# jseppanen/azalea

Measured on AMD Instinct MI355X. Metric: mcts_sims_per_sec, higher is better.
Workload: dtype f16x3 (fp32 operands split hi+lo f16, fp32 accumulate)

## Files before the change

### azalea_amd/csrc/net_kernels.hip

```cpp
#include "net_priv.h"

#ifndef AZX_NET_ABLATE
#define AZX_NET_ABLATE 0
#endif
#ifndef AZX_SAT_TRACK
#define AZX_SAT_TRACK 1
#endif

#include <cmath>
#include <cstdio>
#include <cstdlib>
#include <cstring>
#include <map>
#include <string>
#include <type_traits>
#include <vector>

typedef float f32x16 __attribute__((ext_vector_type(16)));

static thread_local std::string g_net_err;
const char *azx_net_error() { return g_net_err.c_str(); }

int azx_net_fail(int code, const char *msg) {
    g_net_err = msg;
// ... 82 lines not shown
            }
            const float4 *wt = wl + (size_t)tap * (C / 8) * NT * 64;
#pragma unroll 2
            for (int q = 0; q < C / 8; ++q) {
                float4 bfrag[NTW];
#pragma unroll
                for (int n = 0; n < NTW; ++n)
                    bfrag[n] = wt[((size_t)q * NT + (ns * NTW + n)) * 64 + lane];
                float4 afrag[MTW];
#pragma unroll
                for (int m = 0; m < MTW; ++m)
                    afrag[m] = *reinterpret_cast<const float4 *>(src + aoff[m] + 8 * q);
#pragma unroll
                for (int m = 0; m < MTW; ++m)
#pragma unroll
                    for (int n = 0; n < NTW; ++n) {
                        acc[m][n] = __builtin_amdgcn_mfma_f32_32x32x2f32(afrag[m].x, bfrag[n].x, acc[m][n], 0, 0, 0);
                        acc[m][n] = __builtin_amdgcn_mfma_f32_32x32x2f32(afrag[m].y, bfrag[n].y, acc[m][n], 0, 0, 0);
                        acc[m][n] = __builtin_amdgcn_mfma_f32_32x32x2f32(afrag[m].z, bfrag[n].z, acc[m][n], 0, 0, 0);
                        acc[m][n] = __builtin_amdgcn_mfma_f32_32x32x2f32(afrag[m].w, bfrag[n].w, acc[m][n], 0, 0, 0);
                    }
            }
        }
        const bool residual = (layer & 1) != 0;
#pragma unroll
        for (int n = 0; n < NTW; ++n) {
            const int co = (ns * NTW + n) * 32 + li;
            const float bb = P.bias[layer * C + co];
#pragma unroll
            for (int m = 0; m < MTW; ++m) {
#pragma unroll
                for (int r = 0; r < 16; ++r) {
                    const int row = (ms * MTW + m) * 32 + (r & 3) + 8 * (r >> 2) + 4 * lh;
                    if (row < ncells) {
                        float v = acc[m][n][r] + bb;
                        if (residual) v += dst[row * LDW + co];
                        dst[row * LDW + co] = fmaxf(v, 0.0f);
                    }
                }
            }
        }
        __syncthreads();
    }

    for (int b = 0; b < BPB; ++b) {
        const int e = e0 + b;
        if (e >= n_eval) break;
        const float *Xb = lds + (size_t)b * 2 * rows * LDW;
        float4 *out = reinterpret_cast<float4 *>(act_out + (size_t)e * ncells * C);
        for (int idx = tid; idx < ncells * (C / 4); idx += 256) {
            const int pos = idx / (C / 4), c4 = idx - pos * (C / 4);
            out[idx] = *reinterpret_cast<const float4 *>(Xb + pos * LDW + 4 * c4);
        }
    }
}


typedef _Float16 f16x8 __attribute__((ext_vector_type(8)));

__device__ __forceinline__ void split_f16(float v, _Float16 &hi, _Float16 &lo) {
    hi = (_Float16)v;
    lo = (_Float16)(v - (float)hi);
}
__device__ __forceinline__ void split2_f16(float a, float b, uint32_t &hpk, uint32_t &lpk) {
    float la, lb;
    asm("v_cvt_pk_f16_f32 %0, %1, %2" : "=v"(hpk) : "v"(a), "v"(b));
    asm("v_fma_mix_f32 %0, %1, -1.0, %2 op_sel_hi:[1,0,0]" : "=v"(la) : "v"(hpk), "v"(a));
    asm("v_fma_mix_f32 %0, %1, -1.0, %2 op_sel:[1,0,0] op_sel_hi:[1,0,0]" : "=v"(lb) : "v"(hpk), "v"(b));
    asm("v_cvt_pk_f16_f32 %0, %1, %2" : "=v"(lpk) : "v"(la), "v"(lb));
#if AZX_LO_BITS < 10
    lpk = (lpk + LO_RND * 0x10001u) & (LO_MASK * 0x10001u);
#endif
}

#ifdef AZX_NET_STAMP
__device__ unsigned long long g_tower_stamp[10];
#define NT_DECL unsigned long long nt_last = __builtin_amdgcn_s_memtime(), nt_acc[8] = {0, 0, 0, 0, 0, 0, 0, 0}; const unsigned long long nt_rt0 = __builtin_amdgcn_s_memrealtime();
__device__ unsigned long long g_tower_trace[3 * 32768];
#define NT_MARK(r) { const unsigned long long nt_now = __builtin_amdgcn_s_memtime(); nt_acc[r] += nt_now - nt_last; nt_last = nt_now; }
#define NT_FLUSH if (tid == 0) { for (int r_ = 0; r_ < 7; ++r_) atomicAdd(&g_tower_stamp[r_], nt_acc[r_]); atomicAdd(&g_tower_stamp[7], 1ull); atomicAdd(&g_tower_stamp[8], __builtin_amdgcn_s_memrealtime() - nt_rt0); \
    if (blockIdx.x < 32768) { const unsigned hw = __builtin_amdgcn_s_getreg((31 << 11) | 4), xc = __builtin_amdgcn_s_getreg((31 << 11) | 20); \
        g_tower_trace[3 * blockIdx.x] = ((unsigned long long)(xc & 0xf) << 8) | (((hw >> 13) & 7) << 5) | (((hw >> 12) & 1) << 4) | ((hw >> 8) & 0xf); \
        g_tower_trace[3 * blockIdx.x + 1] = nt_rt0; g_tower_trace[3 * blockIdx.x + 2] = __builtin_amdgcn_s_memrealtime(); } }
__device__ unsigned long long g_wide_stamp[10];
#define WT_FLUSH if (lane == 0) { for (int r_ = 0; r_ < 7; ++r_) atomicAdd(&g_wide_stamp[r_], nt_acc[r_]); atomicAdd(&g_wide_stamp[7], 1ull); \
    atomicAdd(&g_wide_stamp[8], __builtin_amdgcn_s_memrealtime() - nt_rt0); }
#else
#define NT_DECL
#define NT_MARK(r)
#define NT_FLUSH
#define WT_FLUSH
#endif

#ifndef F16X3_BPB
#define F16X3_BPB 2
#endif
#ifndef AZX_S16_FENCE
#define AZX_S16_FENCE 1
#endif
typedef float f32x4 __attribute__((ext_vector_type(4)));

__global__ __launch_bounds__(F16X3_BPB * 128, 2) void k_tower_f16x3_s16(NetDev P, const uint8_t *__restrict__ ev_board,
                                                                        const int32_t *__restrict__ n_eval_ptr,
                                                                        int n_eval_host, float *__restrict__ act_out,
                                                                        float *__restrict__ hfeat) {
    constexpr int C = 64, ROWB = 272, MT = 4, NT = 4;
    extern __shared__ __align__(16) unsigned char smem[];
    const int n_eval = n_eval_ptr ? *n_eval_ptr : n_eval_host;
    const int e0 = blockIdx.x * F16X3_BPB;
    if (e0 >= n_eval) return;
    const int tid = threadIdx.x, lane = tid & 63, wave = __builtin_amdgcn_readfirstlane(tid >> 6);
    NT_DECL
    const int wb = wave >> 1, wh = wave & 1;
    const int N = P.N, ncells = P.ncells;
    const int e = e0 + wb;
    const bool live = e < n_eval;
    const int board_b = 128 * ROWB;
    const int zero_off = 0;
    const int x_off = 2 * ROWB + wb * board_b;
    unsigned char *X = smem + x_off;
    const int li = lane & 15, lh = lane >> 4;
    const int lrow = li < 8 ? li ^ 4 : li;
    const int lchunk = 128 * (lh & 1) + 16 * (lh >> 1);

    unsigned long long tapok = 0ull;
    int rbase[MT], ry_[MT], rx_[MT];
#pragma unroll
    for (int m = 0; m < MT; ++m) {
        const int r = 64 * wh + 16 * m + lrow;
        const int ry = r / N, rx = r - ry * N;
        ry_[m] = ry;
        rx_[m] = rx;
        rbase[m] = x_off + r * ROWB + lchunk;
#pragma unroll
        for (int tap = 0; tap < 9; ++tap) {
            const int yy = ry + tap / 3 - 1, xx = rx + tap % 3 - 1;
            if (r < ncells && yy >= 0 && yy < N && xx >= 0 && xx < N) tapok |= 1ull << (tap * 4 + m);
        }
    }
    uint32_t tapok_lo = (uint32_t)tapok, tapok_hi = (uint32_t)(tapok >> 32);
    auto act_offset = [&](int tap, int m) -> int {
        const int delta = ((tap / 3 - 1) * N + (tap % 3 - 1)) * ROWB;
        const uint32_t word = tap < 8 ? tapok_lo : tapok_hi;
        const int mask = (int)(word << (31 - ((tap * 4 + m) & 31))) >> 31;
        return (mask | 0xF0) & (rbase[m] + delta);
    };

    f32x4 res[MT][NT];
    auto load_bias = [&](const float *bias, float4 (&b4)[NT]) {
#pragma unroll
        for (int n = 0; n < NT; ++n) b4[n] = *reinterpret_cast<const float4 *>(bias + 16 * n + 4 * lh);
    };
    float satmax = 0.f;
    auto epilogue = [&](f32x4 (&acc)[MT][NT], const float4 (&bias4)[NT], auto kind_tag) {
        constexpr int kind = decltype(kind_tag)::value;
#pragma unroll
        for (int n = 0; n < NT; ++n) {
            const float4 b4 = bias4[n];
            const float bv[4] = {b4.x, b4.y, b4.z, b4.w};
#pragma unroll
            for (int m = 0; m < MT; ++m) {
                float v4[4];
#pragma unroll
                for (int j = 0; j < 4; ++j) {
                    float v = acc[m][n][j] + bv[j];
                    if (kind == 1) v += res[m][n][j];
                    v = fmaxf(v, 0.0f);
                    if (kind != 0) res[m][n][j] = v;
                    v4[j] = v;
                }
                if (AZX_SAT_TRACK) satmax = fmaxf(fmaxf(satmax, v4[0]), fmaxf(v4[1], fmaxf(v4[2], v4[3])));
                uint2 h4, l4;
                split2_f16(v4[0], v4[1], h4.x, l4.x);
                split2_f16(v4[2], v4[3], h4.y, l4.y);
                unsigned char *pw = X + (64 * wh + 16 * m + lrow) * ROWB + 128 * (lh >> 1) + 16 * n + 8 * (lh & 1);
                *reinterpret_cast<uint2 *>(pw) = h4;
                *reinterpret_cast<uint2 *>(pw + 64) = l4;
            }
        }
    };

    {
        const int NH = N + 2;
        unsigned char *cells = X + 121 * ROWB;
        const uint8_t *bd = ev_board + (size_t)(live ? e : n_eval - 1) * AZX_CELL_STRIDE;
        if (wh == 0) {
            for (int i = lane; i < NH * NH; i += 64) {
                const int y = i / NH - 1, x = i - (y + 1) * NH - 1;
                cells[i] = (y >= 0 && y < N && x >= 0 && x < N) ? bd[y * N + x] : (uint8_t)3;
            }
        }
        for (int i = tid; i < 2 * ROWB / 4; i += F16X3_BPB * 128) reinterpret_cast<uint32_t *>(smem + zero_off)[i] = 0u;
        __syncthreads();
        f32x4 acc[MT][NT];
#pragma unroll
        for (int m = 0; m < MT; ++m)
#pragma unroll
            for (int n = 0; n < NT; ++n) acc[m][n] = f32x4{0.f, 0.f, 0.f, 0.f};
        const uint4 *ws = reinterpret_cast<const uint4 *>(P.Ws16);
        f16x8 wfh[NT], wfl[NT];
#pragma unroll
        for (int n = 0; n < NT; ++n) {
            const uint4 qh = ws[(n * 2) * 64 + lane], ql = ws[(n * 2 + 1) * 64 + lane];
            wfh[n] = *reinterpret_cast<const f16x8 *>(&qh);
            wfl[n] = *reinterpret_cast<const f16x8 *>(&ql);
        }
#pragma unroll
        for (int m = 0; m < MT; ++m) {
            uint32_t onehot = 0u;
            if (64 * wh + 16 * m + lrow < ncells) {
                const unsigned char *c0 = cells + ry_[m] * NH + rx_[m];
#pragma unroll
                for (int tap = 0; tap < 9; ++tap) {
                    const uint32_t v = c0[(tap / 3) * NH + tap % 3];
                    onehot |= (v < 3u ? 1u : 0u) << (3 * tap + v);
                }
            }
            const uint32_t byte = (onehot >> (8 * lh)) & 0xffu;
            uint4 q;
            q.x = ((byte >> 0) & 1u) * 0x3C00u | ((byte >> 1) & 1u) * 0x3C000000u;
            q.y = ((byte >> 2) & 1u) * 0x3C00u | ((byte >> 3) & 1u) * 0x3C000000u;
            q.z = ((byte >> 4) & 1u) * 0x3C00u | ((byte >> 5) & 1u) * 0x3C000000u;
            q.w = ((byte >> 6) & 1u) * 0x3C00u | ((byte >> 7) & 1u) * 0x3C000000u;
            const f16x8 xf = *reinterpret_cast<const f16x8 *>(&q);
#pragma unroll
            for (int n = 0; n < NT; ++n) {
                acc[m][n] = __builtin_amdgcn_mfma_f32_16x16x32_f16(wfh[n], xf, acc[m][n], 0, 0, 0);
                acc[m][n] = __builtin_amdgcn_mfma_f32_16x16x32_f16(wfl[n], xf, acc[m][n], 0, 0, 0);
            }
        }
        float4 sb4[NT];
        load_bias(P.stem_b, sb4);
        __syncthreads();
        epilogue(acc, sb4, std::integral_constant<int, 2>{});
    }
    __syncthreads();
    NT_MARK(0)

    const uint4 *wsrc = reinterpret_cast<const uint4 *>(P.Wh16);
    int stage = 0;
    const int last_stage = P.layers * 18 - 1;
    f16x8 wh_[NT], wl_[NT];
    auto load_w = [&](int st, int nn, int part) {
        const uint4 qq = wsrc[(size_t)min(st, last_stage) * 512 + (nn * 2 + part) * 64 + lane];
        if (part) wl_[nn] = *reinterpret_cast<const f16x8 *>(&qq);
        else wh_[nn] = *reinterpret_cast<const f16x8 *>(&qq);
    };
#pragma unroll
    for (int i = 0; i < 4; ++i) load_w(0, i >> 1, i & 1);
    auto conv_layer = [&](int layer, auto residual_tag) {
        constexpr bool residual = decltype(residual_tag)::value;
        asm volatile("" : "+v"(tapok_lo), "+v"(tapok_hi), "+v"(rbase[0]), "+v"(rbase[1]), "+v"(rbase[2]), "+v"(rbase[3]));
        f32x4 acc[MT][NT];
#pragma unroll
        for (int m = 0; m < MT; ++m)
#pragma unroll
            for (int n = 0; n < NT; ++n) acc[m][n] = f32x4{0.f, 0.f, 0.f, 0.f};
        f16x8 xh[MT], xl[MT];
        auto load_x = [&](int tt, int mm, int part) {
            const unsigned char *pa = smem + act_offset(tt >> 1, mm) + (tt & 1) * 32 + part * 64;
            if (part) xl[mm] = *reinterpret_cast<const f16x8 *>(pa);
            else xh[mm] = *reinterpret_cast<const f16x8 *>(pa);
        };
#pragma unroll
        for (int m = 0; m < MT - 1; ++m) { load_x(0, m, 0); load_x(0, m, 1); }
#pragma unroll
        for (int t = 0; t < 18; ++t) {
#pragma unroll
            for (int h = 0; h < 2; ++h) {
#pragma unroll
                for (int q = 0; q < 24; ++q) {
                    const int m = q / 6, n = 2 * h + (q % 6) / 3, p = q % 3;
                    if (q == 1 || q == 4 || q == 7 || q == 10) {
                        const int idx = (q - 1) / 3;
                        if (h == 0) load_w(stage + t, 2 + (idx >> 1), idx & 1);
                        else load_w(stage + t + 1, idx >> 1, idx & 1);
                    } else if (h == 0 && (q == 13 || q == 16)) {
                        load_x(t, MT - 1, q == 16);
                    } else if (h == 1 && q >= 8 && (q % 6 == 2 || q % 6 == 5)) {
                        if (t + 1 < 18) load_x(t + 1, q / 6 - 1, q % 6 == 5);
                    }
                    const f16x8 wv = p == 1 ? wl_[n] : wh_[n];
                    const f16x8 xv = p == 2 ? xl[m] : xh[m];
                    acc[m][n] = __builtin_amdgcn_mfma_f32_16x16x32_f16(wv, xv, acc[m][n], 0, 0, 0);
#if AZX_S16_FENCE == 2
                    __builtin_amdgcn_sched_barrier(0);
#elif AZX_S16_FENCE == 1
                    if (q % 3 == 2) __builtin_amdgcn_sched_barrier(0);
#elif AZX_S16_FENCE == 3
                    if (q % 6 == 5) __builtin_amdgcn_sched_barrier(0);
#elif AZX_S16_FENCE == 4
                    if (q % 2 == 1) __builtin_amdgcn_sched_barrier(0);
#endif
                }
            }
        }
        stage += 18;
        float4 lb4[NT];
        load_bias(P.bias + layer * C, lb4);
        NT_MARK(2)
        __syncthreads();
        NT_MARK(3)
        epilogue(acc, lb4, std::integral_constant<int, residual ? 1 : 0>{});
        NT_MARK(4)
        __syncthreads();
        NT_MARK(5)
    };
    for (int blk = 0; blk < P.blocks; ++blk) {
        conv_layer(2 * blk, std::false_type{});
        conv_layer(2 * blk + 1, std::true_type{});
    }

    if (hfeat != nullptr) {
        const uint4 *whd = reinterpret_cast<const uint4 *>(P.Whd16);
        f16x8 ah[2], al[2];
#pragma unroll
        for (int ks = 0; ks < 2; ++ks) {
            const uint4 qh = whd[(ks * 2) * 64 + lane], ql = whd[(ks * 2 + 1) * 64 + lane];
            ah[ks] = *reinterpret_cast<const f16x8 *>(&qh);
            al[ks] = *reinterpret_cast<const f16x8 *>(&ql);
        }
        const float4 hb = *reinterpret_cast<const float4 *>(P.hbias16 + 4 * lh);
        const float hbv[4] = {hb.x, hb.y, hb.z, hb.w};
#pragma unroll
        for (int m = 0; m < MT; ++m) {
            f32x4 hacc = f32x4{0.f, 0.f, 0.f, 0.f};
#pragma unroll
            for (int ks = 0; ks < 2; ++ks) {
                const unsigned char *pa = smem + rbase[m] + ks * 32;
                const f16x8 xh = *reinterpret_cast<const f16x8 *>(pa), xl = *reinterpret_cast<const f16x8 *>(pa + 64);
                hacc = __builtin_amdgcn_mfma_f32_16x16x32_f16(ah[ks], xh, hacc, 0, 0, 0);
                hacc = __builtin_amdgcn_mfma_f32_16x16x32_f16(al[ks], xh, hacc, 0, 0, 0);
                hacc = __builtin_amdgcn_mfma_f32_16x16x32_f16(ah[ks], xl, hacc, 0, 0, 0);
            }
            const int row = 64 * wh + 16 * m + lrow;
            if (live && row < ncells) {
#pragma unroll
                for (int r = 0; r < 4; ++r) {
                    const int o = 4 * lh + r;
                    if (o < 6) hfeat[((size_t)e * 6 + o) * ncells + row] = fmaxf(hacc[r] + hbv[r], 0.0f);
                }
            }
        }
    }
    if (live && act_out != nullptr) {
        float *out = act_out + (size_t)e * ncells * C;
#pragma unroll
        for (int m = 0; m < MT; ++m) {
            const int row = 64 * wh + 16 * m + lrow;
            if (row < ncells) {
#pragma unroll
                for (int n = 0; n < NT; ++n)
                    *reinterpret_cast<float4 *>(out + row * C + 16 * n + 4 * lh) =
                        make_float4(res[m][n][0], res[m][n][1], res[m][n][2], res[m][n][3]);
            }
        }
    }
    if (satmax > 65504.0f) atomicOr(P.sat_flag, 1u);
    NT_MARK(6)
    NT_FLUSH
}

#define WIDE_ROWB 272
#define WIDE_MW 3
#define WIDE_NW 2

#ifndef WIDE_STAGE_GROUP
#define WIDE_STAGE_GROUP 6
#endif
#ifndef AZX_WIDE_ABLATE
#define AZX_WIDE_ABLATE 0
#endif

#define WIDE16_MT 6
#define WIDE16_NT 4
struct WideBwdFuse { const unsigned char *mask; const float *raw, *skip; const double *sums; float invN; unsigned int *gmax; };
template <int TRAIN, int NTW = WIDE16_NT>
__device__ __forceinline__ void conv_wide_s16_body(const NetDev &P, int layer, const unsigned short *__restrict__ in,
                                                   unsigned short *out, const unsigned short *resid,
                                                   float *__restrict__ out32,
                                                   const int32_t *__restrict__ n_eval_ptr, int n_eval_host,
                                                   int e_base, int e_end, float unscale, float2 *__restrict__ stat,
                                                   const WideBwdFuse &F = WideBwdFuse{}) {
    constexpr int MT = WIDE16_MT, NT = NTW, ROWB = WIDE_ROWB;
    static_assert(NT == 4 || (NT == 2 && TRAIN != 0), "two tiles per wave: training instantiations only");
    float satmax = 0.f;
    extern __shared__ __align__(16) unsigned char smem[];
    const int n_eval = n_eval_ptr ? *n_eval_ptr : n_eval_host;
    const int C = P.C, N = P.N, ncells = P.ncells;
    const int NCH = C / 64, NT16 = C / 16;
    NT_DECL
    const int e = e_base + blockIdx.y * 8 + (blockIdx.x & 7);
    if (e >= n_eval || e >= e_end) return;
    const int co_base = (blockIdx.x >> 3) * (32 * NT);
    const int tid = threadIdx.x, lane = tid & 63, wave = tid >> 6;
    const int wm = wave & 1, wn = wave >> 1;
    const int row0 = wm ? 80 : 0;
    const int li = lane & 15, lh = lane >> 4;
    const size_t rowg = (size_t)C * 4;
    const unsigned char *gin = reinterpret_cast<const unsigned char *>(in) + (size_t)e * ncells * rowg;
    constexpr int IMG0 = 2 * ROWB;
    const int lrow = li < 8 ? li ^ 4 : li;
    const int lchunk = 128 * (lh & 1) + 16 * (lh >> 1);

    unsigned long long tapok = 0ull;
    int rbase[MT];
#pragma unroll
    for (int m = 0; m < MT; ++m) {
        const int r = row0 + 16 * m + lrow;
        const int ry = r / N, rx = r - ry * N;
        rbase[m] = IMG0 + r * ROWB + lchunk;
#pragma unroll
        for (int tap = 0; tap < 9; ++tap) {
            const int yy = ry + tap / 3 - 1, xx = rx + tap % 3 - 1;
            if (r < ncells && yy >= 0 && yy < N && xx >= 0 && xx < N) tapok |= 1ull << (tap * 6 + m);
        }
    }
    uint32_t tapok_lo = (uint32_t)tapok & 0x3fffffffu, tapok_hi = (uint32_t)(tapok >> 30);
    auto act_offset = [&](int tap, int m) -> int {
        const int delta = ((tap / 3 - 1) * N + (tap % 3 - 1)) * ROWB;
        const uint32_t word = tap < 5 ? tapok_lo : tapok_hi;
        const int bit = (tap < 5 ? tap : tap - 5) * 6 + m;
        const int mask = (int)(word << (31 - bit)) >> 31;
        return (mask | 0xF0) & (rbase[m] + delta);
    };
    if (tid < IMG0 / 4) reinterpret_cast<uint32_t *>(smem)[tid] = 0u;

    auto chan0 = [&](int np) -> int { return co_base + 16 * NT * wn + 32 * np + 8 * lh; };
    f32x4 acc[MT][NT];
    if constexpr (TRAIN != 0) {
#pragma unroll
        for (int m = 0; m < MT; ++m)
#pragma unroll
            for (int n = 0; n < NT; ++n) acc[m][n] = f32x4{0.f, 0.f, 0.f, 0.f};
    } else {
        const unsigned char *gres0 = resid ? reinterpret_cast<const unsigned char *>(resid) + (size_t)e * ncells * rowg : nullptr;
#if AZX_WIDE_ABLATE & 16
        gres0 = nullptr;
#endif
        float bv[2][8];
#pragma unroll
        for (int np = 0; np < 2; ++np) {
            const float4 b0 = *reinterpret_cast<const float4 *>(P.bias + (size_t)layer * C + chan0(np));
// ... 864 lines not shown
            if (b < nb) logit_out[(size_t)(e0 + b) * AZX_CELL_STRIDE + t] = logit;
        }
    }
    __syncthreads();
    if (tid < nb) {
        float acc = 0.f;
        for (int i = 0; i < 64; ++i) acc += h2[i][tid] * P.fc3w[i];
        value_out[e0 + tid] = tanhf(acc + P.fc3b[0]);
    }
    if (!prior_out) return;
    const int lane = tid & 63, wave = tid >> 6;
    for (int b = wave; b < nb; b += 3 * HEADS_KSPLIT) {
        const int e = e0 + b;
        float x[3];
        bool legal[3];
        float mx = -INFINITY;
#pragma unroll
        for (int s = 0; s < 3; ++s) {
            const int cell = s * 64 + lane;
            legal[s] = cell < ncells && ev_board[(size_t)e * AZX_CELL_STRIDE + cell] == 0;
            x[s] = legal[s] ? lg[b][cell] : -INFINITY;
            mx = fmaxf(mx, x[s]);
        }
        mx = wave_max(mx);
        float sum = 0.f;
#pragma unroll
        for (int s = 0; s < 3; ++s) sum += legal[s] ? expf(x[s] - mx) : 0.f;
        const float lse = mx + logf(wave_sum(sum));
        const int flip = ev_flip[e];
#pragma unroll
        for (int s = 0; s < 3; ++s) {
            const int cell = s * 64 + lane;
            if (cell < ncells) {
                const int uc = (flip & 2) ? ncells - 1 - cell : cell;
                int oc = uc;
                if (flip & 1) {
                    const int i = uc / N, j = uc - i * N;
                    oc = (N - 1 - j) * N + (N - 1 - i);
                }
                prior_out[(size_t)e * AZX_CELL_STRIDE + oc] = legal[s] ? expf(x[s] - lse) : 0.f;
            }
        }
    }
}



static int raise_lds_limits() {
    const int cap = 160 * 1024;
    const void *fns[] = {(const void *)k_tower_f16x3_s16, (const void *)k_conv_wide_f16x3_s16,
                         (const void *)k_tower_mfma<64, 4, 2, 1, 2>, (const void *)k_tower_mfma<64, 6, 1, 2, 2>,
                         (const void *)k_tower_mfma<32, 6, 2, 2, 1>, (const void *)k_heads_mfma, (const void *)k_heads};
    for (const void *f : fns)
        if (hipFuncSetAttribute(f, hipFuncAttributeMaxDynamicSharedMemorySize, cap) != hipSuccess)
            return nfail(AZX_EHIP, "net: raising a tower kernel's dynamic LDS limit failed");
    return AZX_OK;
}

int azx_net_create(AzxNet **out, int N, int blocks, int chans, int max_evals, hipStream_t st) {
    if (N < 2 || N > AZX_MAX_BOARD) return nfail(AZX_EINVAL, "net: board size out of range");
    if (blocks < 0 || chans < 1) return nfail(AZX_EINVAL, "net: bad num_blocks/base_chans");
    if (int rc = raise_lds_limits()) return rc;
    AzxNet *net = new AzxNet();
    memset(&net->d, 0, sizeof net->d);
    net->d.N = N;
    net->d.ncells = N * N;
    net->d.C = chans;
    net->d.blocks = blocks;
    net->d.layers = 2 * blocks;
    net->max_evals = max_evals;
    net->stream = st;
    const int ncells = N * N;
    const char *force = getenv("AZX_TOWER");
    const bool want_fp32 = force && !strcmp(force, "fp32");
    if (chans == 64 && ncells <= 121 && blocks >= 1 && !want_fp32) net->tower_variant = 4;
    else if (chans == 64 && ncells <= 128) net->tower_variant = 1;
    else if (chans == 64 && ncells <= 192) net->tower_variant = 2;
    else if (chans == 32 && ncells <= 192) net->tower_variant = 3;
    else if (chans % 128 == 0 && ncells <= 192 && !want_fp32) net->tower_variant = 5;
    net->use_mfma = net->tower_variant != 0;
    { const char *v = getenv("AZX_WIDE_STREAMS"); net->opt_wsplit = std::min(4, std::max(1, v ? atoi(v) : 2)); }
    { const char *v = getenv("AZX_HEADS"); net->opt_heads_mfma = !(v && !strcmp(v, "valu")); }
    { const char *v = getenv("AZX_PACK"); net->pack_on_host = v && !strcmp(v, "host"); }
    {
        char b[260];
        const char *tower = "k_stem_generic + k_conv_generic (VALU)";
        if (net->tower_variant == 4) tower = "k_tower_f16x3_s16";
        else if (net->tower_variant == 5) tower = "k_stem_wide_f16x3 + k_conv_wide_f16x3_s16 per layer";
        else if (net->tower_variant == 1) tower = "k_tower_mfma<64,4,2,1,2> (fp32 MFMA)";
        else if (net->tower_variant == 2) tower = "k_tower_mfma<64,6,1,2,2> (fp32 MFMA)";
        else if (net->tower_variant == 3) tower = "k_tower_mfma<32,6,2,2,1> (fp32 MFMA)";
        const bool hm = net->tower_variant == 4 && net->opt_heads_mfma && ncells <= 128;
        snprintf(b, sizeof b, "%s + %s (%dx%d on %dx%d; AZX_TOWER=%s AZX_WIDE_STREAMS=%d AZX_HEADS=%s AZX_PACK=%s)",
                 tower, hm ? "k_heads_mfma" : "k_heads", blocks, chans, N, N, want_fp32 ? "fp32" : "default",
                 net->opt_wsplit, net->opt_heads_mfma ? "mfma" : "valu", net->pack_on_host ? "host" : "device");
        net->info = b;
    }
    const size_t E = max_evals;
    net->act = nalloc<float>(net, E * ncells * chans);
    net->logit = nalloc<float>(net, E * AZX_CELL_STRIDE);
    if (net->tower_variant == 4) net->hfeat = nalloc<float>(net, E * 6 * ncells);
    net->hb_board = nalloc<uint8_t>(net, E * AZX_CELL_STRIDE);
    net->hb_flip = nalloc<int32_t>(net, E);
    net->hb_value = nalloc<float>(net, E);
    if (!net->use_mfma) {
        net->act2 = nalloc<float>(net, E * ncells * chans);
        net->act3 = nalloc<float>(net, E * ncells * chans);
    }
    if (net->tower_variant == 5) {
        net->wideX = nalloc<unsigned short>(net, E * ncells * chans * 2);
        net->wideY = nalloc<unsigned short>(net, E * ncells * chans * 2);
    }
    if (!net->act || !net->logit || !net->hb_board || !net->hb_flip || !net->hb_value ||
        (!net->use_mfma && (!net->act2 || !net->act3)) || (net->tower_variant == 5 && (!net->wideX || !net->wideY))) {
        azx_net_destroy(net);
        return nfail(AZX_ENOMEM, "net: hipMalloc failed");
    }
    const int bpb = net->tower_variant == 2 ? 1 : 2;
    net->lds_bytes = (size_t)bpb * 2 * (ncells + 1) * (chans + 4) * sizeof(float);
    if (net->tower_variant == 4) net->lds_bytes = (size_t)F16X3_BPB * 128 * 272 + 2 * 272;
    if (net->tower_variant == 5) net->lds_bytes = (size_t)(ncells + 2) * WIDE_ROWB;
    net->d.sat_flag = nalloc<uint32_t>(net, 4);
    if (!net->d.sat_flag || hipDeviceSynchronize() != hipSuccess) {
        azx_net_destroy(net);
        return nfail(AZX_ENOMEM, "net: hipMalloc failed");
    }
    *out = net;
    return AZX_OK;
}

void azx_net_set_stream(AzxNet *net, hipStream_t st, const uint32_t *mask, int words) {
    if (!net) return;
    for (int i = 0; i < 3; ++i) {
        if (net->stream2[i]) { (void)hipStreamSynchronize(net->stream2[i]); (void)hipStreamDestroy(net->stream2[i]); }
        if (net->ev_join[i]) (void)hipEventDestroy(net->ev_join[i]);
        net->stream2[i] = nullptr;
        net->ev_join[i] = nullptr;
    }
    if (net->ev_fork) (void)hipEventDestroy(net->ev_fork);
    net->ev_fork = nullptr;
    net->streams_ok = false;
    net->cu_mask.assign(mask, mask + (mask ? words : 0));
    net->stream = st;
}

void azx_net_destroy(AzxNet *net) {
    if (net) {
        for (int i = 0; i < 3; ++i) {
            if (net->stream2[i]) { (void)hipStreamSynchronize(net->stream2[i]); (void)hipStreamDestroy(net->stream2[i]); }
            if (net->ev_join[i]) (void)hipEventDestroy(net->ev_join[i]);
            net->stream2[i] = nullptr;
            net->ev_join[i] = nullptr;
        }
        if (net->ev_fork) (void)hipEventDestroy(net->ev_fork);
        net->ev_fork = nullptr;
    }
#ifdef AZX_NET_STAMP
    {
        unsigned long long h[10] = {0};
        if (hipMemcpyFromSymbol(h, HIP_SYMBOL(g_wide_stamp), sizeof h) == hipSuccess && h[7]) {
            static const char *nm[6] = {"prologue (bias + residual, setup)", "barrier after staging", "k-loops (MFMA)", "epilogue (stores acknowledged)",
                                        "barrier before staging (skew)", "staging: requests, round trips, LDS writes"};
            unsigned long long tot = 0;
            for (int r = 0; r < 6; ++r) tot += h[r];
            fprintf(stderr, "k_conv_wide_f16x3_s16 stamps over %llu waves: %.0f cycles/wave, shader clock %.0f MHz during the kernel\n",
                    h[7], (double)tot / h[7], h[8] ? 100.0 * (double)tot / (double)h[8] : 0.0);
            for (int r = 0; r < 6; ++r)
                fprintf(stderr, "  %-44s %6.1f%%  %9.0f cycles/wave\n", nm[r], 100.0 * h[r] / tot, (double)h[r] / h[7]);
            unsigned long long z[10] = {0};
            (void)hipMemcpyToSymbol(HIP_SYMBOL(g_wide_stamp), z, sizeof z);
        }
    }
    {
        unsigned long long h[10] = {0};
        if (hipMemcpyFromSymbol(h, HIP_SYMBOL(g_tower_stamp), sizeof h) == hipSuccess && h[7]) {
            static const char *nm[7] = {"stem", "residual load/setup", "k-loop (MFMA)", "barrier after k-loop",
                                        "epilogue", "barrier after epilogue", "output store"};
            unsigned long long tot = 0;
            for (int r = 0; r < 7; ++r) tot += h[r];
            fprintf(stderr, "k_tower_f16x3_s16 stamps over %llu blocks: %.0f cycles/block, shader clock %.0f MHz during the kernel\n",
                    h[7], (double)tot / h[7], h[8] ? 100.0 * (double)tot / (double)h[8] : 0.0);
            for (int r = 0; r < 7; ++r)
                fprintf(stderr, "  %-24s %6.1f%%  %9.0f cycles/block\n", nm[r], 100.0 * h[r] / tot, (double)h[r] / h[7]);
            {
                std::vector<unsigned long long> tr(3 * 32768);
                (void)hipMemcpyFromSymbol(tr.data(), HIP_SYMBOL(g_tower_trace), tr.size() * sizeof(unsigned long long));
                std::map<unsigned long long, std::vector<std::pair<unsigned long long, unsigned long long>>> cu;
                unsigned long long t0 = ~0ull, t1 = 0;
                size_t nblk = 0;
                for (int b = 0; b < 32768; ++b)
                    if (tr[3 * b + 2]) {
                        cu[tr[3 * b]].push_back({tr[3 * b + 1], tr[3 * b + 2]});
                        t0 = std::min(t0, tr[3 * b + 1]);
                        t1 = std::max(t1, tr[3 * b + 2]);
                        ++nblk;
                    }
                double busy = 0, mn = 1e30, mx = 0, lastend_min = 1e30, lastend_max = 0;
                size_t cmin = 1 << 30, cmax = 0;
                for (auto &kv : cu) {
                    double b = 0, le = 0;
                    for (auto &iv : kv.second) { b += (double)(iv.second - iv.first); le = std::max(le, (double)(iv.second - t0)); }
                    busy += b; mn = std::min(mn, b); mx = std::max(mx, b);
                    cmin = std::min(cmin, kv.second.size()); cmax = std::max(cmax, kv.second.size());
                    lastend_min = std::min(lastend_min, le); lastend_max = std::max(lastend_max, le);
                }
                fprintf(stderr, "  last launch: %zu blocks on %zu CUs, span %.1f us, blocks/CU %zu..%zu, mean resident blocks/CU %.2f, "
                        "per-CU block-time %.0f..%.0f us, CU finish %.0f..%.0f us\n", nblk, cu.size(), (t1 - t0) / 100.0, cmin, cmax,
                        busy / ((double)(t1 - t0) * cu.size()), mn / 100.0, mx / 100.0, lastend_min / 100.0, lastend_max / 100.0);
            }
            int nb = -1;
            (void)hipOccupancyMaxActiveBlocksPerMultiprocessor(&nb, (const void *)k_tower_f16x3_s16, F16X3_BPB * 128, net->lds_bytes);
            hipFuncAttributes fa;
            memset(&fa, 0, sizeof fa);
            (void)hipFuncGetAttributes(&fa, (const void *)k_tower_f16x3_s16);
            fprintf(stderr, "  runtime occupancy: %d blocks/CU (dynamic LDS %zu B, static %zu B, %d VGPRs, max threads %d)\n", nb,
                    net->lds_bytes, (size_t)fa.sharedSizeBytes, fa.numRegs, fa.maxThreadsPerBlock);
        }
    }
#endif
    if (!net) return;
    for (void *p : net->allocs) (void)hipFree(p);
    if (net->raw_tab_host) (void)hipHostFree((void *)net->raw_tab_host);
    if (net->wmax_host) (void)hipHostFree((void *)net->wmax_host);
    delete net;
}

bool azx_net_ready(const AzxNet *net) { return net && net->ready; }


static void run_net(AzxNet *net, const uint8_t *boards, const int32_t *flip, const int32_t *n_eval_ptr,
                    int n_host, int max_n, float *logit, float *value, float *prior, hipStream_t st, size_t row0 = 0) {
    const NetDev &d = net->d;
    if (max_n <= 0) return;
    const size_t act_rows = row0 * d.ncells * d.C;
    float *const act = net->act + act_rows;
    float *const act2 = net->act2 ? net->act2 + act_rows : nullptr;
    float *const act3 = net->act3 ? net->act3 + act_rows : nullptr;
    float *const hfeat_rows = net->hfeat ? net->hfeat + row0 * 6 * d.ncells : nullptr;
    const float *hfeat = nullptr;
    if (net->use_mfma) {
        const size_t lds = net->lds_bytes;
        if (net->tower_variant == 4) {
            const dim3 grid((max_n + F16X3_BPB - 1) / F16X3_BPB), block(F16X3_BPB * 128);
            hipLaunchKernelGGL(k_tower_f16x3_s16, grid, block, lds, st, d, boards, n_eval_ptr, n_host, (float *)nullptr, hfeat_rows);
            hfeat = hfeat_rows;
        } else if (net->tower_variant == 5) {
            const dim3 grid(max_n, d.C / 128), block(256);
            hipLaunchKernelGGL(k_stem_wide_f16x3, grid, block, 0, st, d, boards, net->wideX,
                               d.blocks == 0 ? net->act : (float *)nullptr, n_eval_ptr, n_host);
            const int wsplit = net->opt_wsplit;
            {
                int parts = wsplit;
                if (parts > 1 && !net->ev_fork) {
                    bool ok = hipEventCreateWithFlags(&net->ev_fork, hipEventDisableTiming) == hipSuccess;
                    for (int i = 0; i < 3 && ok; ++i)
                        ok = (net->cu_mask.empty() ? hipStreamCreateWithFlags(&net->stream2[i], hipStreamNonBlocking)
                                                   : hipExtStreamCreateWithCUMask(&net->stream2[i], (uint32_t)net->cu_mask.size(), net->cu_mask.data())) == hipSuccess &&
                             hipEventCreateWithFlags(&net->ev_join[i], hipEventDisableTiming) == hipSuccess;
                    net->streams_ok = ok;
                }
                if (parts > 1 && !net->streams_ok) parts = 1;
                const int per = (((max_n + parts - 1) / parts + 7) / 8) * 8;
                if (per >= max_n) parts = 1;
                if (parts > 1 && hipEventRecord(net->ev_fork, st) != hipSuccess) parts = 1;
                for (int part = 1; part < parts; ++part)
                    if (hipStreamWaitEvent(net->stream2[part - 1], net->ev_fork, 0) != hipSuccess) { parts = 1; break; }
                const int per_ok = parts > 1 ? per : max_n;
                for (int part = 0; part < parts; ++part) {
                    hipStream_t s = part ? net->stream2[part - 1] : st;
                    const int e0 = part * per_ok, e1 = std::min(max_n, e0 + per_ok);
                    if (e1 <= e0) continue;
                    const dim3 g(8 * (d.C / 128), (e1 - e0 + 7) / 8);
                    for (int b = 0; b < d.blocks; ++b) {
                        hipLaunchKernelGGL(k_conv_wide_f16x3_s16, g, block, lds, s, d, 2 * b, (const unsigned short *)net->wideX, net->wideY,
                                           (const unsigned short *)nullptr, (float *)nullptr, n_eval_ptr, n_host, e0, e1);
                        hipLaunchKernelGGL(k_conv_wide_f16x3_s16, g, block, lds, s, d, 2 * b + 1, (const unsigned short *)net->wideY, net->wideX,
                                           (const unsigned short *)net->wideX, b == d.blocks - 1 ? net->act : (float *)nullptr, n_eval_ptr, n_host, e0, e1);
                    }
                    if (part) {
                        if (hipEventRecord(net->ev_join[part - 1], s) != hipSuccess ||
                            hipStreamWaitEvent(st, net->ev_join[part - 1], 0) != hipSuccess)
                            (void)hipStreamSynchronize(s);
                    }
                }
            }
        } else if (net->tower_variant == 1) {
            hipLaunchKernelGGL((k_tower_mfma<64, 4, 2, 1, 2>), dim3((max_n + 1) / 2), dim3(256), lds, st, d, boards, n_eval_ptr, n_host, act);
        } else if (net->tower_variant == 2) {
            hipLaunchKernelGGL((k_tower_mfma<64, 6, 1, 2, 2>), dim3(max_n), dim3(256), lds, st, d, boards, n_eval_ptr, n_host, act);
        } else {
            hipLaunchKernelGGL((k_tower_mfma<32, 6, 2, 2, 1>), dim3((max_n + 1) / 2), dim3(256), lds, st, d, boards, n_eval_ptr, n_host, act);
        }
    } else {
        const int grid = 2048;
        hipLaunchKernelGGL(k_stem_generic, dim3(grid), dim3(256), 0, st, d, boards, n_eval_ptr, n_host, max_n, act);
        float *x = act, *y = act2, *z = act3;
        for (int b = 0; b < d.blocks; ++b) {
            hipLaunchKernelGGL(k_conv_generic, dim3(grid), dim3(256), 0, st, d, 2 * b, x, (const float *)nullptr, n_eval_ptr, n_host, max_n, y);
            hipLaunchKernelGGL(k_conv_generic, dim3(grid), dim3(256), 0, st, d, 2 * b + 1, y, x, n_eval_ptr, n_host, max_n, z);
            std::swap(x, z);
        }
        if (x != act)
            (void)hipMemcpyAsync(act, x, (size_t)max_n * d.ncells * d.C * sizeof(float), hipMemcpyDeviceToDevice, st);
    }
    if (hfeat != nullptr && net->opt_heads_mfma && d.ncells <= 128) {
        const size_t hl = std::max((size_t)HM_MB * d.hm_lda, (size_t)HM_MB * AZX_CELL_STRIDE + (size_t)HM_MB * 64) * sizeof(float);
        hipLaunchKernelGGL(k_heads_mfma, dim3((max_n + HM_MB - 1) / HM_MB), dim3(256), hl, st, d, hfeat, boards, flip, n_eval_ptr, n_host, logit, value, prior);
    } else {
        const size_t hl = ((size_t)(6 * d.ncells + 64) * HEADS_BPB + (size_t)HEADS_BPB * AZX_CELL_STRIDE +
                           (size_t)(HEADS_KSPLIT - 1) * (64 + 192) * HEADS_BPB) * sizeof(float);
        hipLaunchKernelGGL(k_heads, dim3((max_n + HEADS_BPB - 1) / HEADS_BPB), dim3(192 * HEADS_KSPLIT), hl, st, d, act, hfeat, boards, flip, n_eval_ptr, n_host, logit, value, prior);
    }
}

const char *azx_net_kernel_info(const AzxNet *net) { return net->info.c_str(); }

int azx_net_check_range(AzxNet *net, hipStream_t st) {
    if (!net || !net->d.sat_flag) return AZX_OK;
    uint32_t flag = 0;
    if (hipMemcpyAsync(&flag, net->d.sat_flag, sizeof flag, hipMemcpyDeviceToHost, st) != hipSuccess ||
        hipStreamSynchronize(st) != hipSuccess)
        return nfail(AZX_EHIP, "net: reading the activation range flag failed");
    if (!flag) return AZX_OK;
    (void)hipMemsetAsync(net->d.sat_flag, 0, sizeof flag, st);
    return nfail(AZX_ERANGE, "net: an activation of the residual tower exceeded the f16 range (65504) of the split-f16 "
                             "kernels -- the evaluations of this call are not valid (AZX_TOWER=fp32 runs the fp32 MFMA tower)");
}
// ... 79 lines not shown
```

### azalea_amd/csrc/net_priv.h

```cpp
#pragma once
#include <hip/hip_runtime.h>
#include <stdint.h>

#include <algorithm>
#include <string>
#include <vector>

#include "net.h"

struct NetDev {
    int N, ncells, C, blocks, layers;
    const float *stemT;
    const float *stem_b;
    const unsigned short *Ws;
    const unsigned short *Ws16, *Wh16;
    const unsigned short *Whd16;
    const float *hbias16;
    const float *Wp;
    const float *Wg;
    const float *bias;
    const float *wv, *bv;
    const float *wp, *bp;
    const float *fc2T, *fc2b;
    const float *fc3w, *fc3b;
    const float *mfcT, *mfcb;
    const float *hmP, *hmV;
    int hm_lda;
    uint32_t *sat_flag;
};

#ifndef AZX_LO_BITS
#define AZX_LO_BITS 10
#endif
#define LO_MASK ((0xFFFFu << (10 - AZX_LO_BITS)) & 0xFFFFu)
#define LO_RND (AZX_LO_BITS < 10 ? (1u << (9 - AZX_LO_BITS)) : 0u)
static inline unsigned short lo_round_bits(unsigned short bits) {
    return (unsigned short)((bits + LO_RND) & LO_MASK);
}

struct AzxNet {
    NetDev d;
    int max_evals = 0;
    bool ready = false;
    bool use_mfma = false;
    hipStream_t stream = nullptr;
    std::vector<void *> allocs;
    float *act = nullptr, *act2 = nullptr, *act3 = nullptr;
    unsigned short *wideX = nullptr, *wideY = nullptr;
    float *logit = nullptr;
    float *hfeat = nullptr;
    uint8_t *hb_board = nullptr;
    int32_t *hb_flip = nullptr;
    float *hb_value = nullptr;
    size_t lds_bytes = 0;
    int tower_variant = 0;
    hipStream_t stream2[3] = {nullptr, nullptr, nullptr};
    std::vector<uint32_t> cu_mask;
    hipEvent_t ev_fork = nullptr, ev_join[3] = {nullptr, nullptr, nullptr};
    bool streams_ok = false;
    int opt_wsplit = 2;
    bool opt_heads_mfma = true;
    std::string info;
    bool pack_on_host = false;
    bool packed_once = false;
    const float **raw_tab = nullptr;
    const float **raw_tab_host = nullptr;
    int raw_slots = 0;
    float *raw_arena = nullptr;
    size_t raw_arena_floats = 0;
    double *fold = nullptr;
    uint32_t *wmax = nullptr;
    uint32_t *wmax_host = nullptr;
    struct PackBuf { std::string name; void *ptr; size_t bytes; };
    std::vector<PackBuf> packs;
};

int azx_net_fail(int code, const char *msg);

template <typename T>
static T *nalloc(AzxNet *net, size_t count) {
    void *p = nullptr;
    if (hipMalloc(&p, std::max<size_t>(count * sizeof(T), 16)) != hipSuccess) return nullptr;
    (void)hipMemset(p, 0, std::max<size_t>(count * sizeof(T), 16));
    net->allocs.push_back(p);
    return reinterpret_cast<T *>(p);
}
```

Baseline: 5.158 million.

## Skip dead-tap MFMAs for last row tile and rebalance wave roles by LDS slot

In the fused f16x3 tower kernel, the last row tile's MFMA triples for the bottom three taps (t>=12) are wrapped in inline asm with a wave-uniform branch. The branch skips them when a ballot shows none of those taps are valid for the wave's rows, so waves covering off-board rows stop doing zero work. It also adds a role flip of the wave-half assignment, chosen by reading the LDS base hardware register, to balance skipped work across SIMDs. The inline asm bypasses compiler scheduling and adds manual nops at the drain point, and a debug placement trace is added under the stamp build.

```diff
diff --git a/azalea_amd/csrc/net_kernels.hip b/azalea_amd/csrc/net_kernels.hip
--- a/azalea_amd/csrc/net_kernels.hip
+++ b/azalea_amd/csrc/net_kernels.hip
@@ -188,6 +188,9 @@
     if (blockIdx.x < 32768) { const unsigned hw = __builtin_amdgcn_s_getreg((31 << 11) | 4), xc = __builtin_amdgcn_s_getreg((31 << 11) | 20); \
         g_tower_trace[3 * blockIdx.x] = ((unsigned long long)(xc & 0xf) << 8) | (((hw >> 13) & 7) << 5) | (((hw >> 12) & 1) << 4) | ((hw >> 8) & 0xf); \
         g_tower_trace[3 * blockIdx.x + 1] = nt_rt0; g_tower_trace[3 * blockIdx.x + 2] = __builtin_amdgcn_s_memrealtime(); } }
+__device__ unsigned int g_tower_place[4 * 32768];
+#define NT_PLACE if (lane == 0 && blockIdx.x < 32768) g_tower_place[4 * blockIdx.x + wave] = 0x80000000u | \
+    (__builtin_amdgcn_s_getreg((11 << 11) | 6) << 8) | ((__builtin_amdgcn_s_getreg((31 << 11) | 4) >> 4) & 3u);
 __device__ unsigned long long g_wide_stamp[10];
 #define WT_FLUSH if (lane == 0) { for (int r_ = 0; r_ < 7; ++r_) atomicAdd(&g_wide_stamp[r_], nt_acc[r_]); atomicAdd(&g_wide_stamp[7], 1ull); \
     atomicAdd(&g_wide_stamp[8], __builtin_amdgcn_s_memrealtime() - nt_rt0); }
@@ -195,6 +198,7 @@
 #define NT_DECL
 #define NT_MARK(r)
 #define NT_FLUSH
+#define NT_PLACE
 #define WT_FLUSH
 #endif
 
@@ -205,11 +209,18 @@
 #define AZX_S16_FENCE 1
 #endif
 typedef float f32x4 __attribute__((ext_vector_type(4)));
+template <int B, int E, typename F>
+__device__ __forceinline__ void static_for(F &&f) {
+    if constexpr (B < E) {
+        f(std::integral_constant<int, B>{});
+        static_for<B + 1, E>(f);
+    }
+}
 
 __global__ __launch_bounds__(F16X3_BPB * 128, 2) void k_tower_f16x3_s16(NetDev P, const uint8_t *__restrict__ ev_board,
                                                                         const int32_t *__restrict__ n_eval_ptr,
                                                                         int n_eval_host, float *__restrict__ act_out,
-                                                                        float *__restrict__ hfeat) {
+                                                                        float *__restrict__ hfeat, int skip_on, int roles) {
     constexpr int C = 64, ROWB = 272, MT = 4, NT = 4;
     extern __shared__ __align__(16) unsigned char smem[];
     const int n_eval = n_eval_ptr ? *n_eval_ptr : n_eval_host;
@@ -217,7 +228,8 @@
     if (e0 >= n_eval) return;
     const int tid = threadIdx.x, lane = tid & 63, wave = __builtin_amdgcn_readfirstlane(tid >> 6);
     NT_DECL
-    const int wb = wave >> 1, wh = wave & 1;
+    const int flip = roles == 2 ? (int)(__builtin_amdgcn_s_getreg((11 << 11) | 6) != 0u) : roles;
+    const int wb = wave >> 1, wh = (wave & 1) ^ flip;
     const int N = P.N, ncells = P.ncells;
     const int e = e0 + wb;
     const bool live = e < n_eval;
@@ -244,6 +256,8 @@
             if (r < ncells && yy >= 0 && yy < N && xx >= 0 && xx < N) tapok |= 1ull << (tap * 4 + m);
         }
     }
+    constexpr unsigned long long DEAD_TAPS = 1ull << (6 * 4 + MT - 1) | 1ull << (7 * 4 + MT - 1) | 1ull << (8 * 4 + MT - 1);
+    const int dead = __builtin_amdgcn_readfirstlane((int)(skip_on != 0 && __builtin_amdgcn_ballot_w64((tapok & DEAD_TAPS) != 0ull) == 0ull));
     uint32_t tapok_lo = (uint32_t)tapok, tapok_hi = (uint32_t)(tapok >> 32);
     auto act_offset = [&](int tap, int m) -> int {
         const int delta = ((tap / 3 - 1) * N + (tap % 3 - 1)) * ROWB;
@@ -370,8 +384,20 @@
         };
 #pragma unroll
         for (int m = 0; m < MT - 1; ++m) { load_x(0, m, 0); load_x(0, m, 1); }
-#pragma unroll
-        for (int t = 0; t < 18; ++t) {
+        auto mfma3_unless_dead = [&](f32x4 &a, const f16x8 &w_hi, const f16x8 &w_lo, const f16x8 &x_hi, const f16x8 &x_lo, int dead_s, auto drain_tag) {
+            if constexpr (decltype(drain_tag)::value)
+                asm volatile("s_cmp_lg_u32 %5, 0\n\ts_cbranch_scc1 1f\n\t"
+                             "v_mfma_f32_16x16x32_f16 %0, %1, %3, %0\n\tv_mfma_f32_16x16x32_f16 %0, %2, %3, %0\n\t"
+                             "v_mfma_f32_16x16x32_f16 %0, %1, %4, %0\n\ts_nop 7\n\ts_nop 7\n\ts_nop 3\n1:"
+                             : "+v"(a) : "v"(w_hi), "v"(w_lo), "v"(x_hi), "v"(x_lo), "s"(dead_s) : "scc");
+            else
+                asm volatile("s_cmp_lg_u32 %5, 0\n\ts_cbranch_scc1 1f\n\t"
+                             "v_mfma_f32_16x16x32_f16 %0, %1, %3, %0\n\tv_mfma_f32_16x16x32_f16 %0, %2, %3, %0\n\t"
+                             "v_mfma_f32_16x16x32_f16 %0, %1, %4, %0\n1:"
+                             : "+v"(a) : "v"(w_hi), "v"(w_lo), "v"(x_hi), "v"(x_lo), "s"(dead_s) : "scc");
+        };
+        auto kstep = [&](auto t_tag) {
+            constexpr int t = decltype(t_tag)::value;
 #pragma unroll
             for (int h = 0; h < 2; ++h) {
 #pragma unroll
@@ -386,9 +412,16 @@
                     } else if (h == 1 && q >= 8 && (q % 6 == 2 || q % 6 == 5)) {
                         if (t + 1 < 18) load_x(t + 1, q / 6 - 1, q % 6 == 5);
                     }
-                    const f16x8 wv = p == 1 ? wl_[n] : wh_[n];
-                    const f16x8 xv = p == 2 ? xl[m] : xh[m];
-                    acc[m][n] = __builtin_amdgcn_mfma_f32_16x16x32_f16(wv, xv, acc[m][n], 0, 0, 0);
+                    if (t >= 12 && m == MT - 1) {
+                        if (p == 0) {
+                            if (t == 17 && q == 21 && h == 1) mfma3_unless_dead(acc[m][n], wh_[n], wl_[n], xh[m], xl[m], dead, std::true_type{});
+                            else mfma3_unless_dead(acc[m][n], wh_[n], wl_[n], xh[m], xl[m], dead, std::false_type{});
+                        }
+                    } else {
+                        const f16x8 wv = p == 1 ? wl_[n] : wh_[n];
+                        const f16x8 xv = p == 2 ? xl[m] : xh[m];
+                        acc[m][n] = __builtin_amdgcn_mfma_f32_16x16x32_f16(wv, xv, acc[m][n], 0, 0, 0);
+                    }
 #if AZX_S16_FENCE == 2
                     __builtin_amdgcn_sched_barrier(0);
 #elif AZX_S16_FENCE == 1
@@ -400,7 +433,8 @@
 #endif
                 }
             }
-        }
+        };
+        static_for<0, 18>([&](auto tc) { kstep(tc); });
         stage += 18;
         float4 lb4[NT];
         load_bias(P.bias + layer * C, lb4);
@@ -465,6 +499,7 @@
     if (satmax > 65504.0f) atomicOr(P.sat_flag, 1u);
     NT_MARK(6)
     NT_FLUSH
+    NT_PLACE
 }
 
 #define WIDE_ROWB 272
@@ -1495,8 +1530,10 @@
     { const char *v = getenv("AZX_WIDE_STREAMS"); net->opt_wsplit = std::min(4, std::max(1, v ? atoi(v) : 2)); }
     { const char *v = getenv("AZX_HEADS"); net->opt_heads_mfma = !(v && !strcmp(v, "valu")); }
     { const char *v = getenv("AZX_PACK"); net->pack_on_host = v && !strcmp(v, "host"); }
+    { const char *v = getenv("AZX_TOWER_SKIP"); net->opt_tower_skip = !(v && !strcmp(v, "0")); }
+    { const char *v = getenv("AZX_TOWER_ROLES"); net->opt_tower_roles = v && !strcmp(v, "0") ? 0 : v && !strcmp(v, "1") ? 1 : 2; }
     {
-        char b[260];
+        char b[320];
         const char *tower = "k_stem_generic + k_conv_generic (VALU)";
         if (net->tower_variant == 4) tower = "k_tower_f16x3_s16";
         else if (net->tower_variant == 5) tower = "k_stem_wide_f16x3 + k_conv_wide_f16x3_s16 per layer";
@@ -1504,9 +1541,11 @@
         else if (net->tower_variant == 2) tower = "k_tower_mfma<64,6,1,2,2> (fp32 MFMA)";
         else if (net->tower_variant == 3) tower = "k_tower_mfma<32,6,2,2,1> (fp32 MFMA)";
         const bool hm = net->tower_variant == 4 && net->opt_heads_mfma && ncells <= 128;
-        snprintf(b, sizeof b, "%s + %s (%dx%d on %dx%d; AZX_TOWER=%s AZX_WIDE_STREAMS=%d AZX_HEADS=%s AZX_PACK=%s)",
+        static const char *const roles_nm[3] = {"0", "1", "auto"};
+        snprintf(b, sizeof b, "%s + %s (%dx%d on %dx%d; AZX_TOWER=%s AZX_WIDE_STREAMS=%d AZX_HEADS=%s AZX_PACK=%s AZX_TOWER_SKIP=%d AZX_TOWER_ROLES=%s)",
                  tower, hm ? "k_heads_mfma" : "k_heads", blocks, chans, N, N, want_fp32 ? "fp32" : "default",
-                 net->opt_wsplit, net->opt_heads_mfma ? "mfma" : "valu", net->pack_on_host ? "host" : "device");
+                 net->opt_wsplit, net->opt_heads_mfma ? "mfma" : "valu", net->pack_on_host ? "host" : "device",
+                 net->opt_tower_skip ? 1 : 0, roles_nm[net->opt_tower_roles]);
         net->info = b;
     }
     const size_t E = max_evals;
@@ -1621,6 +1660,25 @@
                         "per-CU block-time %.0f..%.0f us, CU finish %.0f..%.0f us\n", nblk, cu.size(), (t1 - t0) / 100.0, cmin, cmax,
                         busy / ((double)(t1 - t0) * cu.size()), mn / 100.0, mx / 100.0, lastend_min / 100.0, lastend_max / 100.0);
             }
+            {
+                std::vector<unsigned int> pl(4 * 32768);
+                (void)hipMemcpyFromSymbol(pl.data(), HIP_SYMBOL(g_tower_place), pl.size() * sizeof(unsigned int));
+                std::map<unsigned int, size_t> tuples[2];
+                size_t slot[2] = {0, 0};
+                for (int b = 0; b < 32768; ++b)
+                    if (pl[4 * b] >> 31) {
+                        const int s = ((pl[4 * b] >> 8) & 0xfff) != 0;
+                        unsigned int key = 0;
+                        for (int w = 0; w < 4; ++w) key = key << 4 | (pl[4 * b + w] & 3u);
+                        ++tuples[s][key];
+                        ++slot[s];
+                    }
+                for (int s = 0; s < 2; ++s) {
+                    fprintf(stderr, "  last launch: %zu blocks at LDS base %s, SIMDs of waves 0..3:", slot[s], s ? "> 0" : "0");
+                    for (auto &kv : tuples[s]) fprintf(stderr, " %04x x %zu", kv.first, kv.second);
+                    fprintf(stderr, "\n");
+                }
+            }
             int nb = -1;
             (void)hipOccupancyMaxActiveBlocksPerMultiprocessor(&nb, (const void *)k_tower_f16x3_s16, F16X3_BPB * 128, net->lds_bytes);
             hipFuncAttributes fa;
@@ -1655,7 +1713,8 @@
         const size_t lds = net->lds_bytes;
         if (net->tower_variant == 4) {
             const dim3 grid((max_n + F16X3_BPB - 1) / F16X3_BPB), block(F16X3_BPB * 128);
-            hipLaunchKernelGGL(k_tower_f16x3_s16, grid, block, lds, st, d, boards, n_eval_ptr, n_host, (float *)nullptr, hfeat_rows);
+            hipLaunchKernelGGL(k_tower_f16x3_s16, grid, block, lds, st, d, boards, n_eval_ptr, n_host, (float *)nullptr, hfeat_rows,
+                               net->opt_tower_skip ? 1 : 0, net->opt_tower_roles);
             hfeat = hfeat_rows;
         } else if (net->tower_variant == 5) {
             const dim3 grid(max_n, d.C / 128), block(256);
diff --git a/azalea_amd/csrc/net_priv.h b/azalea_amd/csrc/net_priv.h
--- a/azalea_amd/csrc/net_priv.h
+++ b/azalea_amd/csrc/net_priv.h
@@ -60,6 +60,8 @@
     bool streams_ok = false;
     int opt_wsplit = 2;
     bool opt_heads_mfma = true;
+    bool opt_tower_skip = true;
+    int opt_tower_roles = 2;
     std::string info;
     bool pack_on_host = false;
     bool packed_once = false;
```

Result: no change. 5.200 million, median of 6 (+0.8%).
